# amazon-science/glass-text-spotting

Measured on AMD Instinct MI355X. Metric: images/sec/GPU end-to-end spotting, 1000x1000, ~32 RoIs; 1/2/4/8 GPU scaling, higher is better.
Workload: dtype f32

## Files before the change

glass-text-spotting_amd/csrc/local_stem.hip:

```cpp
#include "common.h"
#include <cstdint>

typedef float f32x16 __attribute__((ext_vector_type(16)));
typedef _Float16 h8s __attribute__((ext_vector_type(8)));
typedef _Float16 h4s __attribute__((ext_vector_type(4)));

namespace {

constexpr int TS = 32;
constexpr int C1W = TS + 2;
constexpr int XW = TS + 4;
constexpr int C1LD = 20;
constexpr int C1LDH = 24;
constexpr int STEM_LDS_BYTES = (XW * XW * 4 + C1W * C1W * C1LD + 16 * 9 * 4) * 4;

struct StemParams {
  const float* x;
  const float* w1;
  const float* b1;
  const float* w2;
  const float* b2;
  void* y;
  int R, H, W, tiles_h, tiles_w;
};

__device__ __forceinline__ float qh(float v) { return (float)(_Float16)v; }
__device__ __forceinline__ float4 qh4(float4 v) { return make_float4(qh(v.x), qh(v.y), qh(v.z), qh(v.w)); }

template <bool H16>
__global__ __launch_bounds__(256, 1) void local_stem_fused_kernel(StemParams p) {
  extern __shared__ __attribute__((aligned(16))) float smem[];
  float4* xin = reinterpret_cast<float4*>(smem);
  float* c1 = smem + XW * XW * 4;
  float4* w1s = reinterpret_cast<float4*>(c1 + C1W * C1W * C1LD);

  const int tid = threadIdx.x, lane = tid & 63;
  const int wv = __builtin_amdgcn_readfirstlane(tid >> 6);
  int b = blockIdx.x;
  const int tw = b % p.tiles_w; b /= p.tiles_w;
  const int th = b % p.tiles_h;
  const int r = b / p.tiles_h;
  const int h0 = th * TS, w0 = tw * TS;

  const float4* xg = reinterpret_cast<const float4*>(p.x) + (long)r * p.H * p.W;
  for (int i = tid; i < XW * XW; i += 256) {
    const int py = i / XW, px = i - py * XW;
    const int hi = h0 - 2 + py, wi = w0 - 2 + px;
    float4 v = make_float4(0.f, 0.f, 0.f, 0.f);
    if ((unsigned)hi < (unsigned)p.H && (unsigned)wi < (unsigned)p.W) v = xg[(long)hi * p.W + wi];
    xin[i] = H16 ? qh4(v) : v;
  }
  if (tid < 16 * 9) {
    const float4 v = reinterpret_cast<const float4*>(p.w1)[tid];
    w1s[tid] = H16 ? qh4(v) : v;
  }
  float4 w2r[H16 ? 1 : 18];
  h8s w2h[H16 ? 9 : 1];
  if constexpr (H16) {
    const float4* w2g = reinterpret_cast<const float4*>(p.w2) + (long)(lane & 31) * 36 + 2 * (lane >> 5);
#pragma unroll
    for (int tap = 0; tap < 9; ++tap) {
      const float4 a = w2g[tap * 4], c = w2g[tap * 4 + 1];
      w2h[tap] = h8s{(_Float16)a.x, (_Float16)a.y, (_Float16)a.z, (_Float16)a.w, (_Float16)c.x, (_Float16)c.y, (_Float16)c.z, (_Float16)c.w};
    }
  } else {
    const float4* w2g = reinterpret_cast<const float4*>(p.w2) + (long)(lane & 31) * 36;
#pragma unroll
    for (int tap = 0; tap < 9; ++tap)
#pragma unroll
      for (int g = 0; g < 2; ++g) w2r[tap * 2 + g] = w2g[tap * 4 + g * 2 + (lane >> 5)];
  }
  __syncthreads();

  {
    constexpr int NPIX = C1W * C1W;
    constexpr int PPT = 5;
    int pix[PPT], base[PPT];
    bool inside[PPT];
#pragma unroll
    for (int q = 0; q < PPT; ++q) {
      const int i = tid + 256 * q;
      pix[q] = i < NPIX ? i : NPIX - 1;
      const int cy = pix[q] / C1W, cx = pix[q] - cy * C1W;
      base[q] = cy * XW + cx;
      const int hi = h0 - 1 + cy, wi = w0 - 1 + cx;
      inside[q] = (unsigned)hi < (unsigned)p.H && (unsigned)wi < (unsigned)p.W;
    }
#pragma unroll
    for (int cg = 0; cg < 4; ++cg) {
      float acc[PPT][4];
      const float4 bv = reinterpret_cast<const float4*>(p.b1)[cg];
#pragma unroll
      for (int q = 0; q < PPT; ++q) { acc[q][0] = bv.x; acc[q][1] = bv.y; acc[q][2] = bv.z; acc[q][3] = bv.w; }
#pragma unroll
      for (int tap = 0; tap < 9; ++tap) {
        const int toff = (tap / 3) * XW + (tap % 3);
        float4 wv4[4];
#pragma unroll
        for (int c = 0; c < 4; ++c) wv4[c] = w1s[(cg * 4 + c) * 9 + tap];
#pragma unroll
        for (int q = 0; q < PPT; ++q) {
          const float4 v = xin[base[q] + toff];
#pragma unroll
          for (int c = 0; c < 4; ++c)
            acc[q][c] = __builtin_fmaf(v.x, wv4[c].x, __builtin_fmaf(v.y, wv4[c].y, __builtin_fmaf(v.z, wv4[c].z, acc[q][c])));
        }
      }
#pragma unroll
      for (int q = 0; q < PPT; ++q) {
        if (tid + 256 * q < NPIX) {
          float4 o = make_float4(fmaxf(acc[q][0], 0.f), fmaxf(acc[q][1], 0.f), fmaxf(acc[q][2], 0.f), fmaxf(acc[q][3], 0.f));
          if (!inside[q]) o = make_float4(0.f, 0.f, 0.f, 0.f);
          if constexpr (H16)
            *reinterpret_cast<h4s*>(reinterpret_cast<_Float16*>(c1) + pix[q] * C1LDH + cg * 4) =
                h4s{(_Float16)o.x, (_Float16)o.y, (_Float16)o.z, (_Float16)o.w};
          else
            *reinterpret_cast<float4*>(&c1[pix[q] * C1LD + cg * 4]) = o;
        }
      }
    }
  }
  __syncthreads();

  f32x16 acc[8];
#pragma unroll
  for (int mb = 0; mb < 8; ++mb)
#pragma unroll
    for (int e = 0; e < 16; ++e) acc[mb][e] = 0.f;
  const int kg = lane >> 5, col = lane & 31;
  if constexpr (H16) {
    const _Float16* a_base = reinterpret_cast<const _Float16*>(c1) + ((8 * wv) * C1W + col) * C1LDH + 8 * kg;
#pragma unroll
    for (int tap = 0; tap < 9; ++tap) {
      const int dy = tap / 3, dx = tap % 3;
#pragma unroll
      for (int mb = 0; mb < 8; ++mb) {
        const h8s af = *reinterpret_cast<const h8s*>(a_base + ((mb + dy) * C1W + dx) * C1LDH);
        acc[mb] = __builtin_amdgcn_mfma_f32_32x32x16_f16(af, w2h[tap], acc[mb], 0, 0, 0);
      }
    }
  } else {
    const float* a_base = c1 + ((8 * wv) * C1W + col) * C1LD + 4 * kg;
#pragma unroll
    for (int tap = 0; tap < 9; ++tap) {
      const int dy = tap / 3, dx = tap % 3;
#pragma unroll
      for (int g = 0; g < 2; ++g) {
        float4 af[8];
#pragma unroll
        for (int mb = 0; mb < 8; ++mb)
          af[mb] = *reinterpret_cast<const float4*>(a_base + ((mb + dy) * C1W + dx) * C1LD + 8 * g);
        const float4 bf = w2r[tap * 2 + g];
#pragma unroll
        for (int s = 0; s < 4; ++s) {
          const float bs = s == 0 ? bf.x : s == 1 ? bf.y : s == 2 ? bf.z : bf.w;
#pragma unroll
          for (int mb = 0; mb < 8; ++mb) {
            const float as = s == 0 ? af[mb].x : s == 1 ? af[mb].y : s == 2 ? af[mb].z : af[mb].w;
            acc[mb] = __builtin_amdgcn_mfma_f32_32x32x2f32(as, bs, acc[mb], 0, 0, 0);
          }
        }
      }
    }
  }

  const float bias = p.b2[col];
  const int Hp = p.H >> 1, Wp = p.W >> 1;
  float* yg = static_cast<float*>(p.y) + (long)r * Hp * Wp * 32;
  _Float16* yh = static_cast<_Float16*>(p.y) + (long)r * Hp * Wp * 32;
#pragma unroll
  for (int q = 0; q < 4; ++q) {
    const int py = (h0 >> 1) + 4 * wv + q;
#pragma unroll
    for (int e = 0; e < 16; e += 2) {
      const float m = fmaxf(fmaxf(acc[2 * q][e], acc[2 * q][e + 1]), fmaxf(acc[2 * q + 1][e], acc[2 * q + 1][e + 1]));
      const int pxc = (e & 3) + 8 * (e >> 2) + 4 * kg;
      const int px = (w0 >> 1) + (pxc >> 1);
      const float o = fmaxf(m + bias, 0.f);
      if constexpr (H16) yh[((long)py * Wp + px) * 32 + col] = (_Float16)o;
      else yg[((long)py * Wp + px) * 32 + col] = o;
    }
  }
}

}

extern "C" int glass_local_stem_supported(int H, int W) { return H > 0 && W > 0 && H % TS == 0 && W % TS == 0; }

static int local_stem_launch(const float* x, const float* w1, const float* b1, const float* w2, const float* b2, void* y, int R,
                             int H, int W, glass_stream_t stream, bool h16) {
  GLASS_CHECK_ARG(x && w1 && b1 && w2 && b2 && y, "glass_local_stem_fused: null pointer");
  GLASS_CHECK_ARG(glass_local_stem_supported(H, W), "glass_local_stem_fused: H=%d, W=%d must be positive multiples of %d", H, W, TS);
  GLASS_CHECK_ARG((((uintptr_t)x | (uintptr_t)w1 | (uintptr_t)b1 | (uintptr_t)w2 | (uintptr_t)y) & 15) == 0,
                  "glass_local_stem_fused: pointers must be 16-byte aligned");
  if (R <= 0) return GLASS_OK;
  StemParams p;
  p.x = x; p.w1 = w1; p.b1 = b1; p.w2 = w2; p.b2 = b2; p.y = y;
  p.R = R; p.H = H; p.W = W; p.tiles_h = H / TS; p.tiles_w = W / TS;
  const long nblk = (long)R * p.tiles_h * p.tiles_w;
  GLASS_CHECK_ARG(nblk <= 0x7fffffffL, "glass_local_stem_fused: too many tiles");
  static int attr_rc = (int)hipFuncSetAttribute(reinterpret_cast<const void*>(local_stem_fused_kernel<false>),
                                                hipFuncAttributeMaxDynamicSharedMemorySize, STEM_LDS_BYTES) |
                       (int)hipFuncSetAttribute(reinterpret_cast<const void*>(local_stem_fused_kernel<true>),
                                                hipFuncAttributeMaxDynamicSharedMemorySize, STEM_LDS_BYTES);
  if (attr_rc != 0) {
    glass_set_error("glass_local_stem_fused: cannot reserve %d bytes of LDS (hip error %d)", STEM_LDS_BYTES, attr_rc);
    return GLASS_EHIP;
  }
  if (h16) hipLaunchKernelGGL(local_stem_fused_kernel<true>, dim3((unsigned)nblk), dim3(256), STEM_LDS_BYTES, (hipStream_t)stream, p);
  else hipLaunchKernelGGL(local_stem_fused_kernel<false>, dim3((unsigned)nblk), dim3(256), STEM_LDS_BYTES, (hipStream_t)stream, p);
  GLASS_CHECK_LAUNCH("glass_local_stem_fused");
  return GLASS_OK;
}

extern "C" int glass_local_stem_fused(const float* x, const float* w1, const float* b1, const float* w2, const float* b2,
                                      float* y, int R, int H, int W, glass_stream_t stream) {
  return local_stem_launch(x, w1, b1, w2, b2, y, R, H, W, stream, false);
}

extern "C" int glass_local_stem_fused_h16(const float* x, const float* w1, const float* b1, const float* w2, const float* b2,
                                          void* y, int R, int H, int W, glass_stream_t stream) {
  return local_stem_launch(x, w1, b1, w2, b2, y, R, H, W, stream, true);
}
```

glass-text-spotting_amd/glass_amd/modeling/fusion/local_feature_extraction.py:

```python
from __future__ import annotations

from typing import Dict, Optional

import torch

from ...utils.module import InferenceModule

from ...checkpoint import fold_conv
from ...ops import native as K
from ...utils.registry import Registry

LOCAL_FEATURE_EXTRACTOR_REGISTRY = Registry("LOCAL_FEATURE_EXTRACTOR")

_LAYERS = ((1, 1), (2, 2), (3, 5), (4, 3))


def build_hybrid_feature_extractor(cfg, input_shape):
    name = cfg.MODEL.LOCAL_FEATURE_EXTRACTOR.NAME
    out_channels = cfg.MODEL.LOCAL_FEATURE_EXTRACTOR.NUM_FEATURES
    return LOCAL_FEATURE_EXTRACTOR_REGISTRY.get(name)(3, out_channels)


@LOCAL_FEATURE_EXTRACTOR_REGISTRY.register()
class ResNetFeatureExtractor(InferenceModule):
    def __init__(self, input_channel, output_channel=512):
        super().__init__()
        assert input_channel == 3
        self.output_channel = output_channel
        self.w: Dict[str, tuple] = {}

    def import_weights(self, sd, device, prefix: str) -> None:
        p = prefix + "ConvNet."
        w = {}
        w["conv0_1"] = fold_conv(sd, p + "conv0_1", p + "bn0_1", device)
        w["conv0_2"] = fold_conv(sd, p + "conv0_2", p + "bn0_2", device)
        for li, nblk in _LAYERS:
            rg = li >= 3
            for b in range(nblk):
                q = f"{p}layer{li}.{b}."
                w[f"l{li}.{b}.conv1"] = fold_conv(sd, q + "conv1", q + "bn1", device, ragged=rg)
                w[f"l{li}.{b}.conv2"] = fold_conv(sd, q + "conv2", q + "bn2", device, ragged=rg)
                if (q + "downsample.0.weight") in sd:
                    w[f"l{li}.{b}.down"] = fold_conv(sd, q + "downsample.0", q + "downsample.1", device)
            if li < 4:
                w[f"conv{li}"] = fold_conv(sd, f"{p}conv{li}", f"{p}bn{li}", device, ragged=rg)
        w["conv4_1"] = fold_conv(sd, p + "conv4_1", p + "bn4_1", device)
        self.w = w

    def forward_nhwc(self, x: torch.Tensor, out: Optional[torch.Tensor] = None, out_coff: int = 0,
                     out_cstride: int = 1) -> torch.Tensor:
        w = self.w
        pools = {1: ((2, 2), (2, 2), (0, 0)), 2: ((2, 2), (2, 2), (0, 0)), 3: ((2, 2), (2, 1), (0, 1))}
        fused_stem = x.shape[0] > 0 and w["conv0_1"][1] is not None and w["conv0_2"][1] is not None and \
            K.local_stem_supported(x, w["conv0_1"][0], w["conv0_2"][0])
        if fused_stem:
            x = K.local_stem_fused(x, *w["conv0_1"], *w["conv0_2"])
        else:
            x = K.conv2d_nhwc(x, *w["conv0_1"], padding=1, relu=1, out_dtype=K.act_dtype(w["conv0_1"][0]))
            x = K.conv2d_nhwc(x, *w["conv0_2"], padding=1, relu=1)
        for li, nblk in _LAYERS:
            if li in pools and x.shape[0] > 0 and not (fused_stem and li == 1):
                x = K.maxpool2d_nhwc(x, *pools[li])
            for b in range(nblk):
                key = f"l{li}.{b}."
                res = K.conv2d_nhwc(x, *w[key + "down"]) if (key + "down") in w else x
                o = K.conv2d_nhwc(x, *w[key + "conv1"], padding=1, relu=1)
                x = K.conv2d_nhwc(o, *w[key + "conv2"], padding=1, relu=1, residual=res, res_mode=1)
            if li < 4:
                x = K.conv2d_nhwc(x, *w[f"conv{li}"], padding=1, relu=1)
        return K.conv2d_nhwc(x, *w["conv4_1"], stride=(2, 1), relu=1, out=out, out_coff=out_coff, out_cstride=out_cstride,
                             out_dtype=torch.float32)

    def forward(self, input: torch.Tensor) -> torch.Tensor:
        x = input.permute(0, 2, 3, 1)
        if x.shape[-1] == 3:
            x = torch.nn.functional.pad(x, (0, 1))
        return self.forward_nhwc(x.contiguous()).permute(0, 3, 1, 2)


LOCAL_FEATURE_EXTRACTOR_REGISTRY.register_unbuilt(
    "ResNetFeatureExtractorV2", "its reference constructor raises NameError (local_feature_extraction.py:36), no config uses it")
```

glass-text-spotting_amd/glass_amd/ops/native.py:

```python
from __future__ import annotations

import collections
import ctypes
import math
import os
import struct
import threading
from typing import List, NamedTuple, Optional, Sequence, Tuple

import numpy as np
import torch

from .._lib import GlassLibraryError, check, lib

c_int, c_float, c_void_p = ctypes.c_int, ctypes.c_float, ctypes.c_void_p


class ConvDesc(ctypes.Structure):
    _fields_ = [(n, c_int) for n in (
        "N", "H", "W", "Cin", "Cout", "KH", "KW", "stride_h", "stride_w", "pad_h", "pad_w", "Ho", "Wo",
        "ldx", "ldy", "y_coff", "y_cstride", "relu", "res_mode", "ldr")]


class RoiAlignDesc(ctypes.Structure):
# ... 55 lines not shown
def conv_out_size(H, W, KH, KW, stride, padding):
    sh, sw = _pair(stride)
    ph, pw = _pair(padding)
    return (H + 2 * ph - KH) // sh + 1, (W + 2 * pw - KW) // sw + 1


_PRECISIONS = ("fp32", "fp16", "fp16s")


_RNN_LAYOUTS = ((1, 1), (2, 1), (2, 2))


def _parse_rnn(v):
    if isinstance(v, str) and v in ("steps", "persistent"):
        return v
    try:
        nd, ng = (int(t) for t in (v if isinstance(v, (tuple, list)) else str(v).split("x")))
    except (TypeError, ValueError):
        nd = ng = -1
    if (nd, ng) not in _RNN_LAYOUTS:
        raise GlassLibraryError(f"unknown recurrent routing {v!r} (steps | persistent | 2x1 | 2x2 | 1x1)")
    return (nd, ng)


def _parse_split(v) -> int:
    try:
        n = int(v)
    except (TypeError, ValueError):
        n = -1
    if n not in (0, 6, 9):
        raise GlassLibraryError(f"unknown 1x1 split routing {v!r} (0 | 9 | 6)")
    return n


def _parse_ragged(v):
    if isinstance(v, str):
        return {"0": False, "strip": True}.get(v, "tiles")
    return bool(v)


class Routing:
    __slots__ = ("precision", "winograd", "f43", "pw", "h16", "local_stem", "stem", "ragged", "pooled_fusion", "rnn", "splitk", "small_grid", "split")

    def __init__(self, precision: Optional[str] = None, winograd: Optional[bool] = None, f43: Optional[bool] = None, pw=None,
                 h16: Optional[bool] = None, local_stem: Optional[bool] = None, stem: Optional[bool] = None,
                 ragged=None, pooled_fusion: Optional[bool] = None, rnn=None,
                 splitk: Optional[bool] = None, small_grid: Optional[bool] = None, split: Optional[int] = None):
        e = os.environ.get
        self.precision = precision or e("GLASS_CONV_PRECISION", "fp32")
        if self.precision not in _PRECISIONS:
            raise GlassLibraryError(f"unknown conv precision {self.precision!r}")
        self.winograd = (e("GLASS_WINOGRAD", "1") != "0") if winograd is None else bool(winograd)
        self.f43 = (e("GLASS_WINOGRAD43", "1") != "0") if f43 is None else bool(f43)
        self.pw = {"0": False, "all": "all"}.get(e("GLASS_POINTWISE", "1"), True) if pw is None else (pw if pw == "all" else bool(pw))
        self.h16 = (e("GLASS_CONV_H16", "1") != "0") if h16 is None else bool(h16)
        self.local_stem = (e("GLASS_LOCAL_STEM", "1") != "0") if local_stem is None else bool(local_stem)
        self.stem = (e("GLASS_BACKBONE_STEM", "1") != "0") if stem is None else bool(stem)
        self.ragged = _parse_ragged(e("GLASS_W43_RAGGED", "tiles") if ragged is None else ragged)
        self.pooled_fusion = (e("GLASS_POOLED_FUSION", "1") != "0") if pooled_fusion is None else bool(pooled_fusion)
        self.rnn = _parse_rnn(e("GLASS_RNN", "1x1")) if rnn is None else _parse_rnn(rnn)
        self.splitk = (e("GLASS_SPLITK", "1") != "0") if splitk is None else bool(splitk)
        self.small_grid = (e("GLASS_SMALL_GRID", "1") != "0") if small_grid is None else bool(small_grid)
        self.split = _parse_split(e("GLASS_PW_SPLIT", "9") if split is None else split)

    def replace(self, **kw) -> "Routing":
        r = Routing.__new__(Routing)
        for k in Routing.__slots__:
            setattr(r, k, kw.pop(k, getattr(self, k)))
        if kw:
            raise TypeError(f"unknown routing fields {sorted(kw)}")
        if r.precision not in _PRECISIONS:
            raise GlassLibraryError(f"unknown conv precision {r.precision!r}")
        r.split = _parse_split(r.split)
        r.rnn = _parse_rnn(r.rnn)
        r.ragged = _parse_ragged(r.ragged)
        return r

    @property
    def act_dtype(self) -> torch.dtype:
        return torch.float16 if self.precision == "fp16s" else torch.float32

    def __repr__(self):
        return "Routing(" + ", ".join(f"{k}={getattr(self, k)!r}" for k in Routing.__slots__) + ")"


_DEFAULT = Routing()
_TLS = threading.local()
_COUNTS = {"on_the_fly": 0}


def default_routing() -> Routing:
    return _DEFAULT


def routing_of(w) -> Routing:
    r = getattr(w, "routing", None)
    return r if r is not None else _DEFAULT


def set_conv_precision(precision: str) -> str:
    if precision not in _PRECISIONS:
        raise GlassLibraryError(f"unknown conv precision {precision!r}")
    prev = _DEFAULT.precision
    _DEFAULT.precision = precision
    return prev


def conv_precision() -> str:
    return _DEFAULT.precision


def act_dtype(w=None) -> torch.dtype:
    return routing_of(w).act_dtype


def last_conv_path() -> str:
    return getattr(_TLS, "last_path", "direct")


def set_winograd(enabled: bool) -> bool:
    prev = _DEFAULT.winograd
    _DEFAULT.winograd = bool(enabled)
    return prev


def set_winograd43(enabled: bool) -> bool:
    prev = _DEFAULT.f43
    _DEFAULT.f43 = bool(enabled)
    return prev


def set_conv_h16(enabled: bool) -> bool:
    prev = _DEFAULT.h16
    _DEFAULT.h16 = bool(enabled)
    return prev


def set_pointwise(enabled: bool) -> bool:
    prev = _DEFAULT.pw
    _DEFAULT.pw = enabled if enabled == "all" else bool(enabled)
    return prev


def set_pw_split(products: int) -> int:
    prev = _DEFAULT.split
    _DEFAULT.split = _parse_split(products)
    return prev


def winograd_pack(w: torch.Tensor, f43=False) -> torch.Tensor:
    _f32c(w, "w")
    Cout, KH, KW, Cin = w.shape
    L = lib()
    if f43 == "col1":
        return w[:, :, 0:2, :].reshape(Cout, 3, 1, 2 * Cin).contiguous()
    if f43 == "h16":
        u = torch.empty((int(L.glass_conv_h16_weight_halves(Cout, KH, KW, Cin)),), dtype=torch.float16, device=w.device)
        check(L.glass_conv_h16_pack_weights(_dev(w, "w"), Cout, KH, KW, Cin, _dev(u), stream_handle()),
              "glass_conv_h16_pack_weights")
        return u
    if f43 == "pws":
        u = torch.empty((int(L.glass_pointwise_split_weight_bytes(Cout, Cin)),), dtype=torch.uint8, device=w.device)
        check(L.glass_pointwise_split_pack_weights(_dev(w, "w"), Cout, Cin, _dev(u), stream_handle()),
              "glass_pointwise_split_pack_weights")
        return u
    if f43 == "pw":
        nf, fn, what = L.glass_pointwise_weight_floats, L.glass_pointwise_pack_weights, "glass_pointwise_pack_weights"
    elif f43:
        nf, fn, what = L.glass_winograd43_weight_floats, L.glass_winograd43_pack_weights, "glass_winograd43_pack_weights"
    else:
        nf, fn, what = L.glass_winograd_weight_floats, L.glass_winograd_pack_weights, "glass_winograd_pack_weights"
    u = torch.empty((int(nf(Cout, Cin)),), dtype=torch.float32, device=w.device)
    check(fn(_dev(w, "w"), Cout, Cin, _dev(u), stream_handle()), what)
    return u


def _wino_workgroups(m: int, N: int, H: int, W: int, Cout: int, wide: bool, body: bool = False) -> int:
    tiles = N * ((H + m - 1) // m) * (W // m if body else (W + m - 1) // m)
    per = (16 if m == 4 else 32) * (1 if wide else 2)
    return -(-tiles // per) * (Cout // 128 if wide else Cout // 64)


def _use_f43(N: int, H: int, W: int, Cout: int, Cin: int, body: bool = False) -> bool:
    t4 = ((H + 3) // 4) * (W // 4 if body else (W + 3) // 4)
    waste = (t4 * 16.0) / (((H + 1) // 2) * ((W + 1) // 2) * 4.0)
    return waste <= 1.25 and _wino_workgroups(4, N, H, W, Cout, Cout % 128 == 0 and Cin % 32 == 0, body) >= 192


NUM_CUS = 256


def _use_split(px: int, Cin: int, Cout: int) -> bool:
    blocks = -(-px // 64) * (Cout // 128)
    if 192 <= blocks < 384 and Cin >= 512:
        return True
    return blocks >= 384 and (Cin >= 128 or px >= 262144)


def _small_grid_3x3(N: int, H: int, W: int, Cout: int, Cin: int, can_body: bool, f43_ok: bool):
    def rounds(blocks):
        return -(-blocks // NUM_CUS)
    cands = []
    wide = Cout % 128 == 0 and Cin % 32 == 0
    for body in ((False, True) if can_body else (False,)):
        strip = 20.0 if body else 0.0
        if f43_ok and (not body or W % 4 == 1):
            blocks = _wino_workgroups(4, N, H, W, Cout, wide, body)
            cands.append((rounds(blocks) * ((10 + 0.34 * Cin) if wide else (9 + 0.56 * Cin)) + strip, "f43", body))
        blocks = _wino_workgroups(2, N, H, W, Cout, wide, body)
        cands.append((rounds(blocks) * ((9 + 0.30 * Cin) if wide else 3.0 * Cin) + strip, "f22", body))
    t, kind, body = min(cands)
    return kind, body, t


def _f43_splitk_plan(N: int, H: int, W: int, Cout: int, Cin: int, can_body: bool):
    if Cout % 128 or Cin % 32:
        return None
    nk = Cin // 32
    best = None
    for body in ((False, True) if (can_body and W % 4 == 1) else (False,)):
        blocks = _wino_workgroups(4, N, H, W, Cout, True, body)
        if blocks > NUM_CUS // 4:
            continue
        for sl in (2, 3, 4, 6, 8, 12, 16, 24, 32):
            if nk % sl or blocks * sl > NUM_CUS:
                continue
            t = -(-(blocks * sl) // NUM_CUS) * (17.0 + 7.5 * nk / sl) + 8.0 + 0.3 * sl + 2.0 * sl * N * H * W * Cout * 4 / 12e6 + (25.0 if body else 0.0)
            if best is None or t < best[2]:
                best = (sl, body, t)
    return best


class ConvWeight:
    __slots__ = ("raw", "packs", "routing", "version")

    def __init__(self, raw: torch.Tensor, routing: Optional[Routing] = None):
        self.raw = _f32c(raw, "w")
        self.packs = {}
        self.routing = routing
        self.version = None if raw.is_inference() else raw._version

    @property
    def shape(self):
        return self.raw.shape

    @property
    def device(self):
        return self.raw.device

    def nbytes(self) -> int:
        return self.raw.numel() * 4 + sum(u.numel() * u.element_size() for u in self.packs.values())


class packing_for:

    def __init__(self, routing):
        self.routing = routing if isinstance(routing, Routing) else Routing(precision=routing)

    def __enter__(self):
        self.prev = getattr(_TLS, "load", None)
        _TLS.load = self.routing
        return self

    def __exit__(self, *exc):
        _TLS.load = self.prev
        return False


def _probe_desc(Cout: int, KH: int, KW: int, Cin: int) -> ConvDesc:
    ph, pw = KH // 2, KW // 2
    return ConvDesc(1, 16, 16, Cin, Cout, KH, KW, 1, 1, ph, pw, 16 + 2 * ph - KH + 1, 16 + 2 * pw - KW + 1, Cin, Cout, 0, 1, 0, 0, 0)


def pack_kinds(Cout: int, KH: int, KW: int, Cin: int, precision: str, stride=1, ragged: bool = False, split: int = 0,
               strip: bool = True) -> list:
    if precision == "all":
        return pack_kinds(Cout, KH, KW, Cin, "fp32", stride, ragged, split=9) + pack_kinds(Cout, KH, KW, Cin, "fp16", stride)
    L, d = lib(), _probe_desc(Cout, KH, KW, Cin)
    kinds = []
    if precision == "fp32":
        if KH == 3 and KW == 3 and _pair(stride) == (1, 1):
            if L.glass_winograd_supported(ctypes.byref(d)):
                kinds.append(False)
            if L.glass_winograd43_supported(ctypes.byref(d)):
                kinds.append(True)
                if ragged and strip and (2 * Cin) % 32 == 0:
                    kinds.append("col1")
        if KH == 1 and KW == 1 and L.glass_pointwise_supported(ctypes.byref(d)):
            kinds.append("pw")
        if split and KH == 1 and KW == 1 and L.glass_pointwise_split_supported(ctypes.byref(d)):
            kinds.append("pws")
    elif Cin % 64 == 0 and L.glass_conv_h16_supported(ctypes.byref(d), 1):
        kinds.append("h16")
    return kinds


def needs_strip_pack(rt: Routing) -> bool:
    return bool(rt.ragged and rt.winograd and (rt.small_grid or rt.ragged != "tiles"))


def prepare_conv_weights(w: torch.Tensor, precision: Optional[str] = None, stride=1, ragged: bool = False) -> ConvWeight:
    if isinstance(w, ConvWeight):
        return w
    if w.dim() == 2:
        w = w.view(w.shape[0], 1, 1, w.shape[1])
    load = getattr(_TLS, "load", None)
# ... 132 lines not shown
    if precision is not None and precision != rt.precision:
        rt = rt.replace(precision=precision)
    _fhc(x, "x")
    N, H, W, ldx = x.shape
    Cout, KH, KW, Cin = wt.shape
    if cin is not None and cin != Cin:
        raise GlassLibraryError(f"cin={cin} does not match weight Cin={Cin}")
    sh, sw = _pair(stride)
    ph, pw = _pair(padding)
    Ho, Wo = (H + 2 * ph - KH) // sh + 1, (W + 2 * pw - KW) // sw + 1
    if out is None:
        out = torch.empty((N, Ho, Wo, Cout), dtype=out_dtype or x.dtype, device=x.device)
    else:
        _fhc(out, "out")
        if tuple(out.shape[:3]) != (N, Ho, Wo):
            raise GlassLibraryError(f"out has shape {tuple(out.shape)}, expected ({N},{Ho},{Wo},*)")
    if out_coff < 0 or out_cstride < 1 or out_coff + (Cout - 1) * out_cstride >= out.shape[3]:
        raise GlassLibraryError(f"output channel window (offset {out_coff}, {Cout} channels, stride {out_cstride}) does not "
                                f"fit the {out.shape[3]} channels of out")
    if residual is not None and residual.shape[-1] < Cout:
        raise GlassLibraryError(f"residual has {residual.shape[-1]} channels, conv produces {Cout}")
    if ldx < Cin:
        raise GlassLibraryError(f"x has {ldx} channels, weight expects {Cin}")
    d = ConvDesc(N, H, W, Cin, Cout, KH, KW, sh, sw, ph, pw, Ho, Wo, ldx, out.shape[3], out_coff, out_cstride, relu,
                 res_mode if residual is not None else 0, residual.shape[-1] if residual is not None else 0)
    if residual is not None:
        _fhc(residual, "residual")
    path, entry, pack, flags, splits, strip, cast = plan_conv(
        d, rt, x_dtype=x.dtype, out_dtype=out.dtype, res_dtype=residual.dtype if residual is not None else None, res_mode=res_mode,
        packs=w.packs if isinstance(w, ConvWeight) else None, forced=winograd, f43k=f43k)
    _TLS.last_path = path
    L = lib()
    xt = x
    if cast:
        xt = torch.empty(x.shape, dtype=torch.float16, device=x.device)
        check(L.glass_cast_f32_to_f16(_dev(x, "x"), _dev(xt), x.numel(), stream_handle()), "glass_cast_f32_to_f16")
    args = [ctypes.byref(d), _dev(xt, "x"), _dev(wt if pack is None else _packed(w, wt, pack), "w"), _opt(bias, "bias"),
            _opt(residual, "residual"), _dev(out, "out")]
    tail = [] if flags is None else [flags]
    if splits:
        nbytes = int(getattr(L, _WORKSPACE_BYTES[entry])(ctypes.byref(d), splits))
        ws = _workspace(nbytes, x.device)
        tail = [splits] + tail + [_dev(ws), nbytes]
    check(getattr(L, entry)(*args, *tail, stream_handle()), entry)
    if strip:
        _last_column_strip(x, _packed(w, wt, "col1"), bias, residual, out, d, out_coff)
    return out


def prepare_dual_weights(w1, w2) -> Optional["ConvWeight"]:
    r1, r2 = _raw(w1), _raw(w2)
    load = getattr(_TLS, "load", None)
    rt = load if load is not None else _DEFAULT
    if (rt.precision != "fp32" or rt.split != 9 or not r1.is_cuda or r1.shape[1:3] != (1, 1) or r2.shape[1:3] != (1, 1) or
            r1.shape[0] != r2.shape[0] or r1.shape[0] % 128 or r1.shape[3] % 32 or r2.shape[3] % 32):
        return None
    cw = ConvWeight(torch.cat([r1, r2], dim=3).contiguous(), routing=load)
    cw.packs["pws"] = winograd_pack(cw.raw, "pws")
    if load is None:
        torch.cuda.current_stream().synchronize()
    return cw


def dual_supported(x1: torch.Tensor, x2: torch.Tensor, w, stride: int = 1, routing: Optional[Routing] = None) -> bool:
    if w is None or not isinstance(w, ConvWeight) or "pws" not in w.packs:
        return False
    rt = routing if routing is not None else routing_of(w)
    if rt.precision != "fp32" or rt.split != 9 or x1.dtype != torch.float32 or x2.dtype != torch.float32:
        return False
    N, H, W, ldx = x1.shape
    Cout, Cin2 = w.raw.shape[0], x2.shape[3]
    Cin1 = w.raw.shape[3] - Cin2
    Ho, Wo = conv_out_size(H, W, 1, 1, stride, 0)
    if Cin1 <= 0 or ldx != Cin1 or tuple(x2.shape[:3]) != (N, Ho, Wo) or not _use_split(N * Ho * Wo, Cin1 + Cin2, Cout):
        return False
    d = ConvDesc(N, H, W, Cin1, Cout, 1, 1, stride, stride, 0, 0, Ho, Wo, ldx, Cout, 0, 1, 0, 0, 0)
    return bool(lib().glass_pointwise_split_dual_supported(ctypes.byref(d), Cin2, x2.shape[3]))


def conv1x1_dual_nhwc(x1: torch.Tensor, x2: torch.Tensor, w: "ConvWeight", bias: Optional[torch.Tensor] = None, *, stride: int = 1,
                      relu: int = 0) -> torch.Tensor:
    _f32c(x1, "x1"); _f32c(x2, "x2")
    N, H, W, ldx = x1.shape
    Cout, Cin2 = w.raw.shape[0], x2.shape[3]
    Cin1 = w.raw.shape[3] - Cin2
    Ho, Wo = conv_out_size(H, W, 1, 1, stride, 0)
    if tuple(x2.shape[:3]) != (N, Ho, Wo) or ldx != Cin1:
        raise GlassLibraryError(f"conv1x1_dual_nhwc: x1 {tuple(x1.shape)} (stride {stride}) and x2 {tuple(x2.shape)} do not share an output grid / weight {tuple(w.raw.shape)}")
    out = torch.empty((N, Ho, Wo, Cout), dtype=torch.float32, device=x1.device)
    d = ConvDesc(N, H, W, Cin1, Cout, 1, 1, stride, stride, 0, 0, Ho, Wo, ldx, Cout, 0, 1, relu, 0, 0)
    _TLS.last_path = "pointwise_split"
    check(lib().glass_conv1x1_pointwise_split_dual_nhwc(ctypes.byref(d), _dev(x1, "x1"), _dev(x2, "x2"), int(Cin2),
                                                        int(x2.shape[3]), _dev(_packed(w, w.raw, "pws"), "w"), _opt(bias, "bias"),
                                                        _dev(out, "out"), stream_handle()),
          "glass_conv1x1_pointwise_split_dual_nhwc")
    return out


def _last_column_strip(x: torch.Tensor, wcol: torch.Tensor, bias, residual, out: torch.Tensor, d: ConvDesc, out_coff: int) -> None:
    N, H, W, Cin, Cout = d.N, d.H, d.W, d.Cin, d.Cout
    assert d.ldx == Cin, "the caller routes only dense inputs here"
    ds = ConvDesc(N, H, 1, 2 * Cin, Cout, 3, 1, 1, 1, 1, 0, H, 1, W * d.ldx, W * d.ldy, (W - 1) * d.ldy + out_coff, 1, d.relu,
                  d.res_mode, W * d.ldr if d.res_mode else 0)
    isz = x.element_size()
    xp = _dev(x, "x") + (W - 2) * d.ldx * isz
    rp = (_dev(residual, "residual") + (W - 1) * d.ldr * residual.element_size()) if (residual is not None and d.res_mode) else None
    check(lib().glass_conv2d_nhwc(ctypes.byref(ds), xp, _dev(wcol, "w"), _opt(bias, "bias"), rp, _dev(out, "out"), stream_handle()),
          "glass_conv2d_nhwc(last column)")


def _splitk_slices(rt: Routing, M: int, Ktot: int, Cin: int, Cout: int, want_time: bool = False):
    if not rt.splitk or rt.precision != "fp32" or Cin % 32 != 0 or M <= 0:
        return (0, float("inf")) if want_time else 0
    nk = Ktot // 32
    if nk < 16:
        return (0, float("inf")) if want_time else 0
    tiles = -(-M // 128) if Cout <= 32 else -(-M // 64) * -(-Cout // 64)

    def t(s):
        wpc = max(1.0, tiles * s / NUM_CUS)
        extra = 0.0 if s == 1 else 2.0 * s * M * Cout * 4 / 4e6 + 5.0 + 0.3 * s
        return nk / s * (0.75 if wpc <= 1.0 else 0.3 + 0.45 * wpc) + extra
    t1 = t(1)
    best, tbest = 0, 0.85 * t1
    for s in (2, 3, 4, 6, 7, 8, 9, 12, 14, 16, 18, 24, 28, 32):
        if nk % s == 0 and nk // s >= 4 and (ts := t(s)) < tbest:
            best, tbest = s, ts
    if want_time:
        return best, (tbest if best else t1)
    return best


def linear(x: torch.Tensor, w, bias: Optional[torch.Tensor] = None, relu: int = 0,
           out: Optional[torch.Tensor] = None, out_dtype: Optional[torch.dtype] = None, precision: Optional[str] = None,
           routing: Optional[Routing] = None) -> torch.Tensor:
    M, K = x.shape
    y = conv2d_nhwc(x.view(M, 1, 1, K), w if isinstance(w, ConvWeight) else w.view(w.shape[0], 1, 1, K), bias, relu=relu,
                    out=None if out is None else out.view(M, 1, 1, -1), out_dtype=out_dtype, precision=precision, routing=routing)
    return y.view(M, -1)


def _raw(w) -> torch.Tensor:
    return w.raw if isinstance(w, ConvWeight) else w


def local_stem_supported(x: torch.Tensor, w1, w2) -> bool:
    rt = routing_of(w1)
    w1, w2 = _raw(w1), _raw(w2)
    return (rt.precision in ("fp32", "fp16s") and rt.local_stem and x.dtype == torch.float32 and
            x.dim() == 4 and x.shape[-1] == 4 and tuple(w1.shape) == (16, 3, 3, 4) and tuple(w2.shape) == (32, 3, 3, 16) and
            bool(lib().glass_local_stem_supported(int(x.shape[1]), int(x.shape[2]))))


def local_stem_fused(x: torch.Tensor, w1, b1: torch.Tensor, w2, b2: torch.Tensor) -> torch.Tensor:
    h16 = routing_of(w1).precision == "fp16s"
    w1, w2 = _raw(w1), _raw(w2)
    for t, n in ((x, "x"), (w1, "w1"), (b1, "b1"), (w2, "w2"), (b2, "b2")):
        _f32c(t, n)
    R, H, W, _ = x.shape
    y = torch.empty((R, H // 2, W // 2, 32), dtype=torch.float16 if h16 else torch.float32, device=x.device)
    fn = lib().glass_local_stem_fused_h16 if h16 else lib().glass_local_stem_fused
    check(fn(_dev(x), _dev(w1), _dev(b1), _dev(w2), _dev(b2), _dev(y), R, H, W, stream_handle()), "glass_local_stem_fused")
    return y


def backbone_stem_supported(x: torch.Tensor, w) -> bool:
    rt = routing_of(w)
    wt = _raw(w)
    return (rt.precision == "fp32" and rt.stem and x.dtype == torch.float32 and x.dim() == 4 and x.shape[-1] == 4 and
            tuple(wt.shape) == (64, 7, 7, 4) and x.shape[0] > 0 and
            bool(lib().glass_backbone_stem_supported(int(x.shape[1]), int(x.shape[2]))))


def backbone_stem_fused(x: torch.Tensor, w, bias: torch.Tensor) -> torch.Tensor:
    wt = _raw(w)
    for t, n in ((x, "x"), (wt, "w"), (bias, "bias")):
        _f32c(t, n)
    N, H, W, _ = x.shape
    y = torch.empty((N, H // 4, W // 4, 64), dtype=torch.float32, device=x.device)
    check(lib().glass_backbone_stem_fused(_dev(x), _dev(wt), _dev(bias), _dev(y), N, H, W, stream_handle()),
          "glass_backbone_stem_fused")
    _TLS.last_path = "fused_stem"
    return y


def maxpool2d_nhwc(x: torch.Tensor, kernel, stride, padding=0) -> torch.Tensor:
    _fhc(x, "x")
    N, H, W, C = x.shape
    KH, KW = _pair(kernel)
    sh, sw = _pair(stride)
    ph, pw = _pair(padding)
    Ho, Wo = (H + 2 * ph - KH) // sh + 1, (W + 2 * pw - KW) // sw + 1
    y = torch.empty((N, Ho, Wo, C), dtype=x.dtype, device=x.device)
    fn = lib().glass_maxpool2d_nhwc_h16 if x.dtype == torch.float16 else lib().glass_maxpool2d_nhwc
    check(fn(_dev(x), _dev(y), N, H, W, C, KH, KW, sh, sw, ph, pw, Ho, Wo, stream_handle()), "glass_maxpool2d_nhwc")
    return y


def pixel_shuffle2x_nhwc(x: torch.Tensor) -> torch.Tensor:
    _f32c(x, "x")
    N, H, W, C4 = x.shape
    C = C4 // 4
    y = torch.empty((N, 2 * H, 2 * W, C), dtype=torch.float32, device=x.device)
    check(lib().glass_pixel_shuffle2x_nhwc(_dev(x), _dev(y), N, H, W, C, stream_handle()), "glass_pixel_shuffle2x_nhwc")
    return y


def mul_(a: torch.Tensor, b: torch.Tensor) -> torch.Tensor:
    _f32c(a, "a"); _f32c(b, "b")
    if a.shape != b.shape:
        raise GlassLibraryError(f"mul_: shapes {tuple(a.shape)} vs {tuple(b.shape)}")
    check(lib().glass_mul_inplace(_dev(a), _dev(b), a.numel(), stream_handle()), "glass_mul_inplace")
    return a


def sigmoid_(x: torch.Tensor) -> torch.Tensor:
    _f32c(x, "x")
    check(lib().glass_sigmoid_inplace(_dev(x), x.numel(), stream_handle()), "glass_sigmoid_inplace")
    return x


def paste_rotated_masks(masks: torch.Tensor, boxes: torch.Tensor, image_hw: Tuple[int, int], threshold: float = 0.5) -> torch.Tensor:
    _f32c(masks, "masks"); _f32c(boxes, "boxes")
    R, M, M2 = masks.shape
    if M != M2:
        raise GlassLibraryError("Only square mask predictions are supported")
    H, W = int(image_hw[0]), int(image_hw[1])
    out = torch.empty((R, H, W), dtype=torch.uint8, device=masks.device)
    if R:
        check(lib().glass_paste_rotated_masks(_dev(masks), _dev(boxes), R, M, H, W, threshold, _dev(out), stream_handle()),
              "glass_paste_rotated_masks")
    return out.view(torch.bool) if threshold >= 0 else out


def preprocess_image(chw: torch.Tensor, mean: Sequence[float], std: Sequence[float], batch: torch.Tensor, n: int) -> None:
    _f32c(chw, "image"); _f32c(batch, "batch")
    _, H, W = chw.shape
    _, Hp, Wp, four = batch.shape
    assert four == 4
    m = (c_float * 3)(*[float(v) for v in mean])
    s = (c_float * 3)(*[float(v) for v in std])
    check(lib().glass_preprocess_image(_dev(chw), H, W, m, s, _dev(batch), int(n), Hp, Wp, stream_handle()),
          "glass_preprocess_image")


def image_u8hwc_to_chw(img: torch.Tensor, out_hw: Tuple[int, int], flip_channels: bool = False) -> torch.Tensor:
    if img.dtype != torch.uint8 or not img.is_contiguous():
        raise GlassLibraryError("image must be contiguous uint8 HWC")
    H, W, C = img.shape
    assert C == 3
    out = torch.empty((3, out_hw[0], out_hw[1]), dtype=torch.float32, device=img.device)
    check(lib().glass_image_u8hwc_to_chw_resized(_dev(img), H, W, _dev(out), int(out_hw[0]), int(out_hw[1]), int(flip_channels),
                                                 stream_handle()), "glass_image_u8hwc_to_chw_resized")
    return out


_PIL_TABLES: dict = {}
_PIL_TABLES_LOCK = threading.Lock()


def _pil_tables(in_size: int, out_size: int, device):
    if in_size == out_size:
        return None, None, 0
    key = (int(in_size), int(out_size), torch.device(device))
    with _PIL_TABLES_LOCK:
        hit = _PIL_TABLES.get(key)
        if hit is None:
            from ..data.transforms import pil_bilinear_coeffs
            k, b = pil_bilinear_coeffs(key[0], key[1])
            if len(_PIL_TABLES) >= 256:
                _PIL_TABLES.clear()
            hit = _PIL_TABLES[key] = (torch.from_numpy(np.array(k)).to(device), torch.from_numpy(np.array(b)).to(device), int(k.shape[1]))
    return hit


def _pil_resize_args(img: torch.Tensor, out_hw: Tuple[int, int]):
    if not isinstance(img, torch.Tensor) or img.dtype != torch.uint8 or not img.is_contiguous() or img.dim() != 3 or img.shape[2] != 3:
        raise GlassLibraryError("image must be contiguous uint8 HWC with 3 channels")
    _dev(img, "image")
    H, W, _ = img.shape
    Ho, Wo = int(out_hw[0]), int(out_hw[1])
    kx, bx, nx = _pil_tables(W, Wo, img.device)
    ky, by, ny = _pil_tables(H, Ho, img.device)
    ptr = lambda t: t.data_ptr() if t is not None else None
    return H, W, Ho, Wo, (ptr(kx), ptr(bx), nx, ptr(ky), ptr(by), ny), (kx, bx, ky, by)


def pil_resize_workspace(H: int, W: int, Ho: int, Wo: int, device) -> Optional[torch.Tensor]:
    nbytes = int(lib().glass_resize_pil_workspace_bytes(int(H), int(W), int(Ho), int(Wo)))
    return torch.empty((nbytes,), dtype=torch.uint8, device=device) if nbytes else None


def pil_resize_u8(img: torch.Tensor, out_hw: Tuple[int, int], workspace: Optional[torch.Tensor] = None) -> torch.Tensor:
    H, W, Ho, Wo, tables, _keep = _pil_resize_args(img, out_hw)
    out = torch.empty((Ho, Wo, 3), dtype=torch.uint8, device=img.device)
    ws = workspace if workspace is not None else pil_resize_workspace(H, W, Ho, Wo, img.device)
    check(lib().glass_resize_u8_pil(_dev(img), H, W, *tables, _opt(ws), ws.numel() * ws.element_size() if ws is not None else 0,
                                    _dev(out), Ho, Wo, stream_handle()), "glass_resize_u8_pil")
    return out


def pil_resize_into_batch(img: torch.Tensor, out_hw: Tuple[int, int], mean: Sequence[float], std: Sequence[float],
                          batch: torch.Tensor, n: int, flip_channels: bool = False,
                          workspace: Optional[torch.Tensor] = None) -> None:
    H, W, Ho, Wo, tables, _keep = _pil_resize_args(img, out_hw)
    _f32c(batch, "batch")
    N, Hp, Wp, four = batch.shape
    assert four == 4
    if not 0 <= int(n) < N:
        raise GlassLibraryError(f"slot {n} outside a batch of {N}")
    m = (c_float * 3)(*[float(v) for v in mean])
    s = (c_float * 3)(*[float(v) for v in std])
    ws = workspace if workspace is not None else pil_resize_workspace(H, W, Ho, Wo, img.device)
    check(lib().glass_resize_u8_pil_into_batch(_dev(img), H, W, *tables, _opt(ws),
                                               ws.numel() * ws.element_size() if ws is not None else 0, Ho, Wo, m, s,
# ... 963 lines not shown
```

Before: 318.8.

## Use Winograd F(2x2,3x3) for second local stem conv with prepacked weights

Result: no change. 321.6 (median of 6 runs) (+0.8%).

```diff
diff --git a/glass-text-spotting_amd/csrc/local_stem.hip b/glass-text-spotting_amd/csrc/local_stem.hip
--- a/glass-text-spotting_amd/csrc/local_stem.hip
+++ b/glass-text-spotting_amd/csrc/local_stem.hip
@@ -1,7 +1,9 @@
 #include "common.h"
+#include "glass_hip_feature_localstem.h"
 #include <cstdint>
 
 typedef float f32x16 __attribute__((ext_vector_type(16)));
+typedef float f32x4 __attribute__((ext_vector_type(4)));
 typedef _Float16 h8s __attribute__((ext_vector_type(8)));
 typedef _Float16 h4s __attribute__((ext_vector_type(4)));
 
@@ -183,9 +185,185 @@
   }
 }
 
+constexpr int WTW = 32, WTH = 16;
+constexpr int WC1W = WTW + 2, WC1H = WTH + 2;
+constexpr int WXW = WTW + 4, WXH = WTH + 4;
+constexpr int STEM_U_FLOATS = 16 * 32 * 16;
+
+struct StemWinoParams {
+  const float* x;
+  const float* w1;
+  const float* b1;
+  const float* u;
+  const float* b2;
+  float* y;
+  int R, H, W, tiles_h, tiles_w;
+};
+
+__global__ __launch_bounds__(256, 2) void local_stem_wino_kernel(StemWinoParams p) {
+  __shared__ __attribute__((aligned(16))) float smem[WXW * WXH * 4 + WC1W * WC1H * C1LD];
+  float* xin = smem;
+  float* c1 = smem + WXW * WXH * 4;
+
+  const int tid = threadIdx.x, lane = tid & 63;
+  const int wv = __builtin_amdgcn_readfirstlane(tid >> 6);
+  const int t = lane & 15, kg = lane >> 4;
+  int b = blockIdx.x;
+  const int tw = b % p.tiles_w; b /= p.tiles_w;
+  const int th = b % p.tiles_h;
+  const int r = b / p.tiles_h;
+  const int h0 = th * WTH, w0 = tw * WTW;
+
+  const float4* xg = reinterpret_cast<const float4*>(p.x) + (long)r * p.H * p.W;
+  for (int i = tid; i < WXW * WXH; i += 256) {
+    const int py = i / WXW, px = i - py * WXW;
+    const int hi = h0 - 2 + py, wi = w0 - 2 + px;
+    float4 v = make_float4(0.f, 0.f, 0.f, 0.f);
+    if ((unsigned)hi < (unsigned)p.H && (unsigned)wi < (unsigned)p.W) v = xg[(long)hi * p.W + wi];
+    reinterpret_cast<float4*>(xin)[i] = v;
+  }
+  float w1a[7];
+  int xoff[7];
+#pragma unroll
+  for (int s = 0; s < 7; ++s) {
+    const int kk = 4 * s + kg, tap = kk / 3, ch = kk - 3 * tap;
+    const bool real = kk < 27;
+    w1a[s] = real ? p.w1[(t * 9 + tap) * 4 + ch] : 0.f;
+    xoff[s] = real ? ((tap / 3) * WXW + tap % 3) * 4 + ch : 0;
+  }
+  const f32x4 bias1 = {p.b1[4 * kg], p.b1[4 * kg + 1], p.b1[4 * kg + 2], p.b1[4 * kg + 3]};
+  const int cb = wv & 1;
+  f32x4 ur[16];
+#pragma unroll
+  for (int xi = 0; xi < 16; ++xi) ur[xi] = reinterpret_cast<const f32x4*>(p.u)[(xi * 2 + cb) * 64 + lane];
+  __syncthreads();
+
+  {
+    constexpr int NPIX = WC1W * WC1H;
+    constexpr int NGRP = (NPIX + 15) / 16;
+#pragma unroll 1
+    for (int g0 = wv; g0 < NGRP; g0 += 8) {
+      int i[2], pix[2], cy[2], cx[2];
+      const float* src[2];
+      f32x4 acc[2];
+#pragma unroll
+      for (int h = 0; h < 2; ++h) {
+        i[h] = 16 * (g0 + 4 * h) + t;
+        pix[h] = i[h] < NPIX ? i[h] : NPIX - 1;
+        cy[h] = pix[h] / WC1W; cx[h] = pix[h] - cy[h] * WC1W;
+        src[h] = xin + (cy[h] * WXW + cx[h]) * 4;
+        acc[h] = bias1;
+      }
+#pragma unroll
+      for (int s = 0; s < 7; ++s)
+#pragma unroll
+        for (int h = 0; h < 2; ++h) {
+          float xv = src[h][xoff[s]];
+          if (s == 6 && kg == 3) xv = 0.f;
+          acc[h] = __builtin_amdgcn_mfma_f32_16x16x4f32(w1a[s], xv, acc[h], 0, 0, 0);
+        }
+#pragma unroll
+      for (int h = 0; h < 2; ++h) {
+        const int hi = h0 - 1 + cy[h], wi = w0 - 1 + cx[h];
+        const bool inside = (unsigned)hi < (unsigned)p.H && (unsigned)wi < (unsigned)p.W;
+        f32x4 o;
+#pragma unroll
+        for (int c = 0; c < 4; ++c) o[c] = inside ? fmaxf(acc[h][c], 0.f) : 0.f;
+        if (i[h] < NPIX) *reinterpret_cast<f32x4*>(&c1[pix[h] * C1LD + 4 * kg]) = o;
+      }
+    }
+  }
+  __syncthreads();
+
+  const int c0 = 16 * cb + 4 * kg;
+  const f32x4 bias = {p.b2[c0], p.b2[c0 + 1], p.b2[c0 + 2], p.b2[c0 + 3]};
+  const int Hp = p.H >> 1, Wp = p.W >> 1;
+  float* yg = p.y + (long)r * Hp * Wp * 32;
+#pragma unroll 1
+  for (int gi = 0; gi < 4; ++gi) {
+    const int g = 4 * (wv >> 1) + gi;
+    const float* src = c1 + ((2 * g) * WC1W + 2 * t) * C1LD + 4 * kg;
+    f32x4 d[4][4];
+#pragma unroll
+    for (int i = 0; i < 4; ++i)
+#pragma unroll
+      for (int j = 0; j < 4; ++j) d[i][j] = *reinterpret_cast<const f32x4*>(src + (i * WC1W + j) * C1LD);
+#pragma unroll
+    for (int j = 0; j < 4; ++j) {
+      const f32x4 a0 = d[0][j] - d[2][j], a1 = d[1][j] + d[2][j], a2 = d[2][j] - d[1][j], a3 = d[1][j] - d[3][j];
+      d[0][j] = a0; d[1][j] = a1; d[2][j] = a2; d[3][j] = a3;
+    }
+    f32x4 y00, y01, y10, y11;
+#pragma unroll
+    for (int i = 0; i < 4; ++i) {
+      const f32x4 v[4] = {d[i][0] - d[i][2], d[i][1] + d[i][2], d[i][2] - d[i][1], d[i][1] - d[i][3]};
+      f32x4 m[4];
+#pragma unroll
+      for (int j = 0; j < 4; ++j) {
+        f32x4 a = {0.f, 0.f, 0.f, 0.f};
+#pragma unroll
+        for (int s = 0; s < 4; ++s) a = __builtin_amdgcn_mfma_f32_16x16x4f32(ur[i * 4 + j][s], v[j][s], a, 0, 0, 0);
+        m[j] = a;
+      }
+      const f32x4 r0 = m[0] + m[1] + m[2], r1 = m[1] - m[2] - m[3];
+      if (i == 0) { y00 = r0; y01 = r1; }
+      if (i == 1) { y00 += r0; y01 += r1; y10 = r0; y11 = r1; }
+      if (i == 2) { y00 += r0; y01 += r1; y10 -= r0; y11 -= r1; }
+      if (i == 3) { y10 -= r0; y11 -= r1; }
+    }
+    f32x4 o;
+#pragma unroll
+    for (int c = 0; c < 4; ++c)
+      o[c] = fmaxf(fmaxf(fmaxf(y00[c], y01[c]), fmaxf(y10[c], y11[c])) + bias[c], 0.f);
+    const int py = (h0 >> 1) + g, px = (w0 >> 1) + t;
+    *reinterpret_cast<f32x4*>(yg + ((long)py * Wp + px) * 32 + c0) = o;
+  }
+}
+
+__global__ void local_stem_pack_weights_kernel(const float* __restrict__ w2, float* __restrict__ u) {
+  const int o = blockIdx.x * blockDim.x + threadIdx.x;
+  if (o >= STEM_U_FLOATS) return;
+  const int s = o & 3, lane = (o >> 2) & 63, cb = (o >> 8) & 1, xi = o >> 9;
+  const int co = 16 * cb + (lane & 15), ci = 4 * (lane >> 4) + s;
+  const double G[4][3] = {{1.0, 0.0, 0.0}, {0.5, 0.5, 0.5}, {0.5, -0.5, 0.5}, {0.0, 0.0, 1.0}};
+  const int i = xi >> 2, j = xi & 3;
+  double acc = 0.0;
+#pragma unroll
+  for (int a = 0; a < 3; ++a)
+#pragma unroll
+    for (int c = 0; c < 3; ++c) acc += G[i][a] * G[j][c] * (double)w2[((co * 3 + a) * 3 + c) * 16 + ci];
+  u[o] = (float)acc;
+}
+
 }
 
 extern "C" int glass_local_stem_supported(int H, int W) { return H > 0 && W > 0 && H % TS == 0 && W % TS == 0; }
+
+extern "C" size_t glass_local_stem_weight_floats(void) { return STEM_U_FLOATS; }
+
+extern "C" int glass_local_stem_pack_weights(const float* w2, float* u_packed, glass_stream_t stream) {
+  GLASS_CHECK_ARG(w2 && u_packed, "glass_local_stem_pack_weights: null pointer");
+  hipLaunchKernelGGL(local_stem_pack_weights_kernel, dim3(STEM_U_FLOATS / 256), dim3(256), 0, (hipStream_t)stream, w2, u_packed);
+  GLASS_CHECK_LAUNCH("glass_local_stem_pack_weights");
+  return GLASS_OK;
+}
+
+extern "C" int glass_local_stem_fused_packed(const float* x, const float* w1, const float* b1, const float* u_packed, const float* b2,
+                                             float* y, int R, int H, int W, glass_stream_t stream) {
+  GLASS_CHECK_ARG(x && w1 && b1 && u_packed && b2 && y, "glass_local_stem_fused_packed: null pointer");
+  GLASS_CHECK_ARG(glass_local_stem_supported(H, W), "glass_local_stem_fused_packed: H=%d, W=%d must be positive multiples of %d", H, W, TS);
+  GLASS_CHECK_ARG((((uintptr_t)x | (uintptr_t)w1 | (uintptr_t)u_packed | (uintptr_t)y) & 15) == 0,
+                  "glass_local_stem_fused_packed: x, w1, u_packed and y must be 16-byte aligned");
+  if (R <= 0) return GLASS_OK;
+  StemWinoParams p;
+  p.x = x; p.w1 = w1; p.b1 = b1; p.u = u_packed; p.b2 = b2; p.y = y;
+  p.R = R; p.H = H; p.W = W; p.tiles_h = H / WTH; p.tiles_w = W / WTW;
+  const long nblk = (long)R * p.tiles_h * p.tiles_w;
+  GLASS_CHECK_ARG(nblk <= 0x7fffffffL, "glass_local_stem_fused_packed: too many tiles");
+  hipLaunchKernelGGL(local_stem_wino_kernel, dim3((unsigned)nblk), dim3(256), 0, (hipStream_t)stream, p);
+  GLASS_CHECK_LAUNCH("glass_local_stem_fused_packed");
+  return GLASS_OK;
+}
 
 static int local_stem_launch(const float* x, const float* w1, const float* b1, const float* w2, const float* b2, void* y, int R,
                              int H, int W, glass_stream_t stream, bool h16) {
diff --git a/glass-text-spotting_amd/glass_amd/modeling/fusion/local_feature_extraction.py b/glass-text-spotting_amd/glass_amd/modeling/fusion/local_feature_extraction.py
--- a/glass-text-spotting_amd/glass_amd/modeling/fusion/local_feature_extraction.py
+++ b/glass-text-spotting_amd/glass_amd/modeling/fusion/local_feature_extraction.py
@@ -34,6 +34,7 @@
         w = {}
         w["conv0_1"] = fold_conv(sd, p + "conv0_1", p + "bn0_1", device)
         w["conv0_2"] = fold_conv(sd, p + "conv0_2", p + "bn0_2", device)
+        K.prepare_local_stem_weights(w["conv0_2"][0])
         for li, nblk in _LAYERS:
             rg = li >= 3
             for b in range(nblk):
diff --git a/glass-text-spotting_amd/glass_amd/ops/native.py b/glass-text-spotting_amd/glass_amd/ops/native.py
--- a/glass-text-spotting_amd/glass_amd/ops/native.py
+++ b/glass-text-spotting_amd/glass_amd/ops/native.py
@@ -231,6 +231,12 @@
     _f32c(w, "w")
     Cout, KH, KW, Cin = w.shape
     L = lib()
+    if f43 == "lstem":
+        if (Cout, KH, KW, Cin) != (32, 3, 3, 16):
+            raise ValueError(f"the local stem packs a [32,3,3,16] weight, not {tuple(w.shape)}")
+        u = torch.empty((int(L.glass_local_stem_weight_floats()),), dtype=torch.float32, device=w.device)
+        check(L.glass_local_stem_pack_weights(_dev(w, "w"), _dev(u), stream_handle()), "glass_local_stem_pack_weights")
+        return u
     if f43 == "col1":
         return w[:, :, 0:2, :].reshape(Cout, 3, 1, 2 * Cin).contiguous()
     if f43 == "h16":
@@ -669,15 +675,30 @@
             bool(lib().glass_local_stem_supported(int(x.shape[1]), int(x.shape[2]))))
 
 
+def prepare_local_stem_weights(w2) -> None:
+    if isinstance(w2, ConvWeight) and w2.raw.is_cuda and tuple(w2.shape) == (32, 3, 3, 16):
+        rt = w2.routing if w2.routing is not None else _DEFAULT
+        if rt.precision == "fp32" and rt.local_stem:
+            w2.packs["lstem"] = winograd_pack(w2.raw, "lstem")
+            if getattr(_TLS, "load", None) is None:
+                torch.cuda.current_stream().synchronize()
+
+
 def local_stem_fused(x: torch.Tensor, w1, b1: torch.Tensor, w2, b2: torch.Tensor) -> torch.Tensor:
     h16 = routing_of(w1).precision == "fp16s"
+    w2cw = w2
     w1, w2 = _raw(w1), _raw(w2)
     for t, n in ((x, "x"), (w1, "w1"), (b1, "b1"), (w2, "w2"), (b2, "b2")):
         _f32c(t, n)
     R, H, W, _ = x.shape
     y = torch.empty((R, H // 2, W // 2, 32), dtype=torch.float16 if h16 else torch.float32, device=x.device)
-    fn = lib().glass_local_stem_fused_h16 if h16 else lib().glass_local_stem_fused
-    check(fn(_dev(x), _dev(w1), _dev(b1), _dev(w2), _dev(b2), _dev(y), R, H, W, stream_handle()), "glass_local_stem_fused")
+    if h16:
+        check(lib().glass_local_stem_fused_h16(_dev(x), _dev(w1), _dev(b1), _dev(w2), _dev(b2), _dev(y), R, H, W, stream_handle()),
+              "glass_local_stem_fused_h16")
+    else:
+        u = _packed(w2cw, w2, "lstem")
+        check(lib().glass_local_stem_fused_packed(_dev(x), _dev(w1), _dev(b1), _dev(u), _dev(b2), _dev(y), R, H, W, stream_handle()),
+              "glass_local_stem_fused_packed")
     return y
 
 
diff --git a/include/glass_hip_feature_localstem.h b/include/glass_hip_feature_localstem.h
--- /dev/null
+++ b/include/glass_hip_feature_localstem.h
@@ -0,0 +1,18 @@
+#ifndef GLASS_HIP_FEATURE_LOCALSTEM_H
+#define GLASS_HIP_FEATURE_LOCALSTEM_H
+
+#include "glass_hip.h"
+
+#ifdef __cplusplus
+extern "C" {
+#endif
+
+size_t glass_local_stem_weight_floats(void);
+int glass_local_stem_pack_weights(const float* w2, float* u_packed, glass_stream_t stream);
+int glass_local_stem_fused_packed(const float* x, const float* w1, const float* b1, const float* u_packed, const float* b2,
+                                  float* y, int R, int H, int W, glass_stream_t stream);
+
+#ifdef __cplusplus
+}
+#endif
+#endif
```
